# 0417keito/JEN-1-pytorch

Hardware: AMD Instinct MI355X
Metric: denoiser steps/sec (B=8, 128x1500 latents) (higher is better)
Workload: dtype bf16; 1 GPU; configs[1] full JEN-1 1D-UNet (296.5M params), B=8 per GPU, latents 128x1500, 100-step DDIM schedule, eta=1 (the reference's default, gdm.py:28: every step adds sigma * noise; the per-step noise is a table drawn before the timed region and READ inside it), no CFG (CFG dropout off: sampling), hipGraph-replayed step; per sampling run and outside the timed region: the text K/V projection and the time; global_batch=8, seq_len=1500, parallelism=replicas x1 (independent samples)

## Files before the change

### include/jen1_deep.h

```cpp
#ifndef JEN1_DEEP_H
#define JEN1_DEEP_H

#include <stdint.h>

#include "jen1_hip.h"

#ifdef __cplusplus
extern "C" {
#endif

#define JEN1_DEEP_GEMM 0
#define JEN1_DEEP_ATTN 1
#define JEN1_DEEP_STATS 2
#define JEN1_DEEP_TILE 3

#define JEN1_DEEP_MAX_SRC 4
#define JEN1_DEEP_MAX_SEG 12
#ifndef JEN1_DEEP_THREADS
#define JEN1_DEEP_THREADS 512
#endif
#define JEN1_DEEP_BLOB_BYTES 4096
#define JEN1_DEEP_MAX_PHASES 256
#ifndef JEN1_DEEP_SHARDS
#define JEN1_DEEP_SHARDS 32
// ... 38 lines not shown
  int32_t pro_mode, norm_C, gn_groups, gn_cpg, gran;
  float inv_count, gn_eps, inv_vpr, inv_Lin, inv_Lout, inv_groups;
  int32_t p_ld;
  int32_t lvn, lvr;
  int32_t out_C, ps_f, ps_off, L_y, y_brows, y_row0, ld_y, ld_res, act, y_f32;
  int32_t part_off, stat_off, red_off;
  jen1_deep_src src[JEN1_DEEP_MAX_SRC];
  int32_t red_bytes;
  int32_t Lp, Hb, zrow, Rtot;
  int32_t lS, lvpg, lgroups;
  int32_t mrep;
  int32_t live_mask;
  const float* wscale;
  int32_t n_chunks, Lc;
  float inv_nchunks;
  int32_t pad_hot_;
  const float* edge_bias;
} jen1_deep_hot;

typedef struct jen1_deep_tile {
  const float* st[2];
  float* out_part;
  int32_t st_tiles[2], st_nfg[2];
  int32_t st_live;
  int32_t cmain;
  int32_t taps, pad_left;
  int32_t tb, tiles_t;
  int32_t BM, mblocks, MF;
  int32_t NF, KS, kch, rows_in;
  int32_t out_nfg, out_cps;
  int32_t tab_off, red_off;
// ... 25 lines not shown
} jen1_deep_phase;

int jen1_deep_phase_size(void);
int jen1_deep_has_chunks(void);

int jen1_deep_phase_conv(const jen1_conv_args* a, int nb_max, jen1_deep_phase* out);

int jen1_deep_phase_attention(const void* q, const void* k, const void* v, void* out_t, const int32_t* kv_row, const void* kv_extra,
                              const int32_t* extra_row, const int32_t* extra_step, int ld_extra, int kx_off, int vx_off, int B, int H,
                              int d, int Nq, int Nk, int ldq, int q_off, int ldkv, int k_off, int v_off, int ldo, int causal,
                              float scale, const float* ln_u, const float* ln_b, int ln_C, float ln_eps, int finish_q,
                              int finish_kv, int kv_live , int dtype, jen1_deep_phase* out);

int jen1_deep_phase_stats(const void* x, float* stats, int B, int L, int ld, int dtype, jen1_deep_phase* out);

int jen1_deep_phase_tile(const jen1_conv_args* a, int tb, int bm, const float* st0, int st0_tiles, int st0_nfg, const float* st1,
                         int st1_tiles, int st1_nfg, int st_live, float* out_part, int out_nfg, jen1_deep_phase* out);
int jen1_deep_tile_count(int L_out, int tb, int M, int bm);

int jen1_deep_link(jen1_deep_phase* phases, int n_phases, int nwg, void* blobs, void* headers);
int jen1_deep_blob_bytes(void);

int jen1_deep_poison(const void* table_dev, int n, uint32_t* sync, void* stream);
int jen1_deep_poison_zero(const void* table_dev, int n, uint32_t* sync, void* zero_ptr, int64_t zero_bytes, void* stream);

int64_t jen1_deep_sync_bytes(int n_phases);

int jen1_deep_num_workgroups(void);

int jen1_deep_run(const void* blobs_dev, const void* headers_dev, int n_phases, uint32_t* sync, int nwg, int lds_bytes, int dtype,
// ... 14 lines not shown
```

### include/jen1_hip.h

```cpp
#ifndef JEN1_HIP_H
#define JEN1_HIP_H

#include <stdint.h>

#ifdef __cplusplus
extern "C" {
#endif

#define JEN1_F32 0
#define JEN1_BF16 1
#define JEN1_FP8 2

#define JEN1_PRO_NONE 0
#define JEN1_PRO_GN 1
#define JEN1_PRO_GN_SILU 2
#define JEN1_PRO_LN 3
#define JEN1_PRO_SILU 4

#define JEN1_ACT_NONE 0
#define JEN1_ACT_GELU 1

#define JEN1_CFG_W64x64 0
#define JEN1_CFG_W128x64 1
#define JEN1_CFG_S16x64 2
// ... 58 lines not shown
  int32_t splitk;
  int32_t cfg;
  int32_t direct;
  const void* zeros;
  int32_t tiles_t;
  float inv_tiles_t, inv_tb;
  const int32_t* film_step;
  const float* ln_u;
  int32_t ln_fold;
  int32_t nseg;
  jen1_conv_seg seg[JEN1_MAX_SEG];
  int32_t m_split;
  int32_t k_split;
  const float* w_scale;
  int32_t live_mask;
  int32_t reserved_;
  const float* edge_bias;
} jen1_conv_args;

int jen1_conv_gemm(const jen1_conv_args* args, void* stream);
int64_t jen1_conv_gemm_lds_bytes(const jen1_conv_args* args);
int jen1_cfg_bm(int cfg);
int jen1_cfg_bn(int cfg);

typedef struct jen1_norm_args {
  const void* x0; const void* x1; void* y;
  const float* gn_stats0; const float* gn_stats1;
  const float* gamma; const float* beta;
  const float* film; const int32_t* film_row;
  const float* ln_rowstats;
  int32_t dtype, mode, B, L, c0, c1, ld0, ld1, ld_y;
// ... 168 lines not shown
```

### jen-1-pytorch_amd/csrc/deep_kernel.hip

```cpp
#include <cstdlib>
#include <type_traits>
#ifdef JEN1_DEEP_EXP_PLAIN
#define JEN1_LIVE_LOAD(p) (*(p))
#endif
#include "live_words.h"
#include "mfma_frag.h"
#include "jen1_deep.h"

namespace {

constexpr int NT = JEN1_DEEP_THREADS;
constexpr int NW = NT / 64;
constexpr int SHARDS = JEN1_DEEP_SHARDS;
static_assert(SHARDS >= 1 && SHARDS <= 63, "one wave polls the shards and the error word");
constexpr int SHW = JEN1_DEEP_SHARD_WORDS;
constexpr int QCHUNK = 32;
#ifndef JEN1_DEEP_ATTN_LIVE_VEC
#define JEN1_DEEP_ATTN_LIVE_VEC 2
#endif

template <typename T> struct Mode { typedef T G; };
template <> struct Mode<fp8_t> { typedef bf16_t G; };
constexpr float P_SCALE = JEN1_FP8_P_SCALE;

// ... 1933 lines not shown
  JEN1_CHECK(!a->ln_fold && !a->row_scale, "deep conv: LayerNorm-fold epilogue / row scale are not supported by the persistent kernel");
  JEN1_CHECK(a->c0 > 0 && a->c0 % 32 == 0 && a->c1 % 32 == 0 && a->M % 16 == 0, "deep conv: channels must be multiples of 32, M of 16");
  JEN1_CHECK(a->taps >= 1 && a->stride >= 1 && a->B >= 1 && a->L_in >= 1 && a->L_out >= 1, "deep conv: bad geometry");
  JEN1_CHECK(a->nseg >= 0 && a->nseg <= JEN1_DEEP_MAX_SRC - 2, "deep conv: at most %d extra K segments", JEN1_DEEP_MAX_SRC - 2);
  JEN1_CHECK(a->taps + a->nseg <= JEN1_DEEP_MAX_SEG, "deep conv: too many K segments");
  const int es = a->dtype == JEN1_F32 ? 4 : (a->dtype == JEN1_FP8 ? 1 : 2);
  const int maxv = a->dtype == JEN1_F32 ? JEN1_DEEP_MAXV_F : JEN1_DEEP_MAXV_B;
  jen1_deep_phase& p = *out;
  memset(&p, 0, sizeof(p));
  p.h.wscale = a->dtype == JEN1_FP8 ? a->w_scale : nullptr;
  p.h.live_mask = a->live_mask;
  p.h.kind = JEN1_DEEP_GEMM;
  p.h.dtype = a->dtype;
  p.h.dep = -1;
  int ns = 0, coff = 0;
  p.h.src[ns++] = jen1_deep_src{a->x0, a->ld0, a->c0, 0, 1.0f};
  coff = a->c0;
  if (a->c1) {
    JEN1_CHECK(a->x1, "deep conv: c1 without x1");
    p.h.src[ns++] = jen1_deep_src{a->x1, a->ld1, a->c1, coff, a->src1_scale};
    coff += a->c1;
  }
  const int cmain = coff;
  int G = 0, nseg = 0;
  for (int tap = 0; tap < a->taps; ++tap) {
    G += cmain / 32;
    p.seg[nseg++] = jen1_deep_seg{0, tap - a->pad_left, G, 0};
  }
  for (int s = 0; s < a->nseg; ++s) {
    const jen1_conv_seg& e = a->seg[s];
    JEN1_CHECK(e.x && e.kch > 0 && e.ld >= 32 * e.kch, "deep conv: bad extra segment %d", s);
// ... 189 lines not shown
  jen1_deep_phase& p = *out;
  memset(&p, 0, sizeof(p));
  p.h.kind = JEN1_DEEP_STATS;
  p.h.dtype = dtype;
  p.h.dep = -1;
  p.sx = x; p.sstats = stats; p.sL = L; p.sld = ld;
  p.scpf = ld / JEN1_FINE_GROUPS;
  p.sgran = p.scpf >= 8 ? 8 : p.scpf;
  p.h.B = B;
  p.h.n_units = B;
  const int vpr = ld / 8, sub = 8 / p.sgran;
  p.h.lds_bytes = align16i((JEN1_DEEP_THREADS / vpr) * vpr * sub * 8);
  return 0;
}

extern "C" int jen1_deep_tile_count(int L_out, int tb, int M, int bm) {
  if (tb < 1 || bm < 1) return 0;
  return ceil_div(L_out, tb) * ceil_div(M, bm);
}

extern "C" int jen1_deep_phase_tile(const jen1_conv_args* a, int tb, int bm, const float* st0, int st0_tiles, int st0_nfg, const float* st1,
                                    int st1_tiles, int st1_nfg, int st_live, float* out_part, int out_nfg, jen1_deep_phase* out) {
  JEN1_CHECK(a && out, "deep tile: null pointer");
  JEN1_CHECK(a->dtype == JEN1_F32 || a->dtype == JEN1_BF16, "deep tile: dtype must be float32 or bf16 (the JEN1_FP8 mode runs the long levels in bf16)");
  JEN1_CHECK(a->x0 && a->w && a->y, "deep tile: null tensor");
  JEN1_CHECK(!a->edge_bias, "deep tile: an edge bias is an option of the deep GEMM phases only");
  JEN1_CHECK(a->pro_mode == JEN1_PRO_NONE || a->pro_mode == JEN1_PRO_GN || a->pro_mode == JEN1_PRO_GN_SILU, "deep tile: prologue %d is not supported", a->pro_mode);
  JEN1_CHECK(!a->ln_fold && !a->row_scale && !a->out_rowstats && a->act == JEN1_ACT_NONE && a->m_split == 0, "deep tile: LayerNorm / row scale / activation / dual range are not tile options");
  JEN1_CHECK(a->c0 > 0 && a->c0 % 32 == 0 && a->c1 % 32 == 0 && a->M % 16 == 0, "deep tile: channels must be multiples of 32, M of 16");
  JEN1_CHECK(a->taps >= 1 && a->stride >= 1 && a->B >= 1 && a->L_in >= 1 && a->L_out >= 1, "deep tile: bad geometry");
// ... 96 lines not shown
  p.tl.tab_off = tile_b;
  p.tl.red_off = tile_b + align16i(8 * cmain);
  const int tot = p.tl.red_off + (2 * (JEN1_DEEP_THREADS / 64) * 64 + 128) * 4;
  JEN1_CHECK(tot <= LDS_BUDGET, "deep tile: %d B of LDS", tot);
  p.h.lds_bytes = tot;
  p.h.n_units = p.tl.mblocks * a->B * p.tl.tiles_t;
  JEN1_CHECK(p.h.n_units < (1 << 20), "deep tile: too many units");
  p.tl.inv_tiles_t = 1.0f / (float)p.tl.tiles_t;
  p.tl.inv_bt = 1.0f / (float)(a->B * p.tl.tiles_t);
  p.h.inv_vpr = 1.0f / (float)(coff / 8);
  p.h.inv_Lin = 1.0f / (float)a->L_in;
  p.h.inv_Lout = 1.0f / (float)a->L_out;
  return 0;
}

extern "C" int jen1_deep_link(jen1_deep_phase* phases, int n_phases, int nwg, void* blobs, void* headers) {
  JEN1_CHECK(phases && blobs && headers && n_phases >= 1 && nwg >= 1, "deep link: bad arguments");
  JEN1_CHECK(n_phases <= JEN1_DEEP_MAX_PHASES, "deep link: %d phases (at most %d)", n_phases, JEN1_DEEP_MAX_PHASES);
  int lds = 0, rot = 0, units_before = 0;
  unsigned char* bl = reinterpret_cast<unsigned char*>(blobs);
  int32_t* hd = reinterpret_cast<int32_t*>(headers);
  memset(bl, 0, (size_t)n_phases * BLOB);
  for (int p = 0; p < n_phases; ++p) {
    jen1_deep_phase& P = phases[p];
    if (P.h.kind == JEN1_DEEP_GEMM && P.h.mrep == 1 && !getenv("JEN1_DEEP_NO_MREP")) {
      int mrep = 1;
      const char* cap_s = getenv("JEN1_DEEP_UNIT_CAP");
      int cap = cap_s ? atoi(cap_s) : nwg;
      static const int cap_attn = getenv("JEN1_DEEP_CAP_BEFORE_ATTN") ? atoi(getenv("JEN1_DEEP_CAP_BEFORE_ATTN")) : 0;
      if (cap_attn > 0 && p + 1 < n_phases && phases[p + 1].h.kind == JEN1_DEEP_ATTN && cap_attn < cap) cap = cap_attn;
      const int nch = P.h.n_chunks < 1 ? 1 : P.h.n_chunks;
      while (mrep < 8 && (P.h.MT / mrep) * P.h.groups_n * nch > cap && P.h.MT % (2 * mrep) == 0 && P.h.mt_split % (2 * mrep) == 0) mrep *= 2;
      if (mrep > 1 && P.h.lds_bytes + P.h.red_bytes <= LDS_BUDGET) {
        P.h.mrep = mrep;
        P.h.n_units = (P.h.MT / mrep) * P.h.groups_n * nch;
        P.h.lds_bytes += P.h.red_bytes;
      }
    }
    P.h.dep = p - 1;
    P.h.dep_units = p ? phases[p - 1].h.n_units : 0;
    P.h.rot = rot % nwg;
    rot += ((P.h.n_units + 7) / 8) * 8;
    lds = P.h.lds_bytes > lds ? P.h.lds_bytes : lds;
    unsigned char* b = bl + (size_t)p * BLOB;
    memcpy(b, &P, sizeof(P));
    hd[4 * p + 0] = P.h.n_units; hd[4 * p + 1] = P.h.rot; hd[4 * p + 2] = P.h.kind; hd[4 * p + 3] = units_before;
    units_before += P.h.n_units;
    if (P.h.kind != JEN1_DEEP_GEMM) continue;
    int16_t* cnt = reinterpret_cast<int16_t*>(b + TAB_OFF);
    int32_t* runs = reinterpret_cast<int32_t*>(b + TAB_OFF + 64);
    const int tmax = (P.h.L_out - 1) * P.h.stride;
    int k0 = 0;
    for (int s = 0; s < P.h.nseg; ++s) {
      const int sb = s ? P.seg[s - 1].gend : 0, se = P.seg[s].gend, sh = P.seg[s].shift;
      if (!(tmax + sh >= 0 && sh < P.h.L_in)) continue;
      const bool low = P.h.mt_split && sb < P.h.g_split;
      JEN1_CHECK(!low || se <= P.h.g_split, "deep link: phase %d: the dual-range split must fall on a segment boundary", p);
      const int Ls = se - sb;
      for (int w = 0; w < NW; ++w) {
        const int i0 = ((w - k0) % NW + NW) % NW;
        if (i0 >= Ls) continue;
        const int n = (Ls - i0 + NW - 1) / NW;
        const int r = cnt[2 * NW + w];
        JEN1_CHECK(r < MAXRUN, "deep link: phase %d has more than %d runs per wave", p, MAXRUN);
        int32_t* e = runs + ((size_t)w * MAXRUN + r) * 4;
        e[0] = sb + i0; e[1] = n; e[2] = P.seg[s].coff + i0 * 32; e[3] = sh;
        cnt[w] = (int16_t)(cnt[w] + n);
        cnt[2 * NW + w] = (int16_t)(r + 1);
        if (low) { cnt[NW + w] = cnt[w]; cnt[3 * NW + w] = cnt[2 * NW + w]; }
      }
      k0 += Ls;
    }
    if (!P.h.mt_split) for (int w = 0; w < NW; ++w) { cnt[NW + w] = cnt[w]; cnt[3 * NW + w] = cnt[2 * NW + w]; }
    const int pf = P.h.dtype == JEN1_F32 ? JEN1_DEEP_PF_F : JEN1_DEEP_PF_B;
    int32_t* slots = reinterpret_cast<int32_t*>(b + SLOT_OFF);
    int32_t* curs = reinterpret_cast<int32_t*>(b + CUR_OFF);
    for (int w = 0; w < NW; ++w) {
      const int32_t* rw = runs + (size_t)w * MAXRUN * 4;
      const int nr = cnt[2 * NW + w], tot = cnt[w];
// ... 8 lines not shown
        if (i + 1 == pf) {
          int r2 = r, l2 = left, g2 = g, c2 = col, s2 = sh;
          if (i + 1 < tot) {
            if (--l2 > 0) { g2 += NW; c2 += NW * 32; }
            else if (r2 + 1 < nr) { ++r2; l2 = rw[r2 * 4 + 1]; g2 = rw[r2 * 4]; c2 = rw[r2 * 4 + 2]; s2 = rw[r2 * 4 + 3]; }
          }
          curs[w * 8 + 0] = r2; curs[w * 8 + 1] = l2; curs[w * 8 + 2] = g2; curs[w * 8 + 3] = c2; curs[w * 8 + 4] = s2;
        }
        if (i + 1 < tot) next();
      }
    }
  }
  return lds + WS_OFF;
}

namespace {
struct PoisonEntry {
  unsigned long long ptr, bytes;
};
__global__ __launch_bounds__(256) void poison_kernel(const PoisonEntry* __restrict__ tab, unsigned* __restrict__ sync, int n_tab, void* zero_ptr,
                                                      unsigned long long zero_bytes) {
  if ((int)blockIdx.y >= n_tab) {
    uint4* z = reinterpret_cast<uint4*>(zero_ptr);
    const size_t n = zero_bytes >> 4;
    const size_t nblk = (size_t)gridDim.x * (gridDim.y - n_tab), blk = (size_t)(blockIdx.y - n_tab) * gridDim.x + blockIdx.x;
    for (size_t i = blk * 256 + threadIdx.x; i < n; i += nblk * 256) z[i] = make_uint4(0u, 0u, 0u, 0u);
    return;
  }
  const PoisonEntry e = tab[blockIdx.y];
  uint4* p = reinterpret_cast<uint4*>(e.ptr);
// ... 90 lines not shown
```

### jen-1-pytorch_amd/jen1_amd/engine.py

```python
from __future__ import annotations

import contextlib
import ctypes as C
import math
import weakref
import os
import time
from collections import namedtuple
from typing import Callable, Dict, List, Optional, Tuple

import torch

from . import lib as L
from .config import ResSpec, TransformerSpec, UNetSpec
from .packing import (conv_weight_to_gemm, convT_weight_to_gemm, ff_out_matrix, fold_layernorm, fold_linear_into_upsample,
                      o1q2_matrix, o2f1_matrix, pack_gemm_weight, pqkv_matrix, s1q2_matrix)

FG = 32


def _ceil_to(x: int, m: int) -> int:
    return (x + m - 1) // m * m


# ... 163 lines not shown

    def nbytes(self) -> int:
        return sum(t.numel() * t.element_size() for t in self.w.values())

    def fold_up(self, uname: str) -> Tuple[torch.Tensor, torch.Tensor, torch.Tensor]:
        key = f"{uname}.upf"
        if key not in self.w:
            f, wt, b_up, wp, bp, w2, b2 = self._fold_src[uname]
            wm, bm = ff_out_matrix(wp, bp, w2, b2)
            wf, b_mid, b_first, b_last = fold_linear_into_upsample(wt, b_up, f, wm, bm)
            self.w[key] = pack_gemm_weight(wf, self.dtype)
            self.v[f"{key}.bias"] = b_mid.float().contiguous()
            self.v[f"{key}.edge"] = torch.stack([b_first, b_last], 0).float().contiguous()
        return self.w[key], self.v[f"{key}.bias"], self.v[f"{key}.edge"]

    def fp8(self, w: torch.Tensor) -> Tuple[torch.Tensor, torch.Tensor]:
        hit = self._fp8.get(id(w))
        if hit is not None and hit[0] is w:
            return hit[1], hit[2]
        MT = w.shape[-3]
        wf = w.reshape(-1, MT, 4, 16, 8).to(torch.float32)
        amax = wf.abs().amax(dim=(0, 2, 4))
        scale = (amax / 448.0).clamp_min(1e-20)
        q = (wf / scale[None, :, None, :, None]).to(torch.float8_e4m3fn).view(torch.uint8).reshape(-1, MT, 64, 8).contiguous()
        scale = scale.reshape(-1).contiguous()
        self._fp8[id(w)] = (w, q, scale)
        return q, scale


def _bgemm_parts(groups):
    if all(n0 % 128 == 0 and N % 128 == 0 for _, _, n0, N, _ in groups):
        return [groups]
    return [[gr] for gr in groups]


def _group_align(part) -> int:
    n_lo = part[0][2]
    return 256 if all((n0 - n_lo) % 256 == 0 and N % 256 == 0 for _, _, n0, N, _ in part) else 128


def parse_fold_up(s: str) -> Optional[frozenset]:
    s = s.strip().lower()
    if s in ("", "1", "all", "on"):
        return None
    if s in ("0", "off", "none"):
        return frozenset()
    return frozenset(int(v) for v in s.split(",") if v.strip())


class DeepIneligible(Exception):
    """a layer does not fit the persistent deep-level kernel (LDS / staging registers / unsupported option)"""


class DeepProgram:

    _static_owner: Dict[str, "weakref.ref"] = {}

    def __init__(self, eng, leader: Optional["DeepProgram"] = None, err: Optional[torch.Tensor] = None):
# ... 62 lines not shown
    def _new(self):
        return (C.c_char * self.dsize)()

    def _add(self, buf, rc, label, out, kind="gemm", part=None):
        if rc != 0:
            msg = self.lib.jen1_last_error()
            raise self.ineligible(f"{label}: {msg.decode() if msg else 'does not fit'}")
        self.bufs.append(buf)
        self.labels.append(label)
        self.outs.append(out)
        self.kinds.append(kind)
        self._note_output(out)
        if part is not None:
            self._produced.setdefault(part.untyped_storage().data_ptr(), part)

    def add_conv(self, a: "L.ConvArgs", label: str, out, nb_max: int = 0):
        buf = self._new()
        self._add(buf, self.lib.jen1_deep_phase_conv(C.byref(a), nb_max, C.cast(buf, C.c_void_p)), label, out)

    def add_tile(self, a: "L.ConvArgs", tb: int, bm: int, st, out_part, out_nfg: int, label: str, out):
        buf = self._new()
        st = list(st) + [None] * (2 - len(st))
        p = [(0, 0, 0) if e is None else (e[0], e[1], e[2]) for e in st]
        live = sum(1 << k for k, e in enumerate(st) if e is not None and e[3])
        rc = self.lib.jen1_deep_phase_tile(C.byref(a), tb, bm, p[0][0] or None, p[0][1], p[0][2], p[1][0] or None, p[1][1], p[1][2], live,
                                           _ptr(out_part), out_nfg, C.cast(buf, C.c_void_p))
        self._add(buf, rc, label, out, kind="tile", part=out_part)

    def add_attention(self, args, label: str, out):
        buf = self._new()
        self._add(buf, self.lib.jen1_deep_phase_attention(*args, C.cast(buf, C.c_void_p)), label, out, kind="attn")

    def add_stats(self, x: "Act", stats: torch.Tensor, label: str):
# ... 138 lines not shown
    def __call__(self, stream: int) -> None:
        self.fn(stream)


def conv_traffic(taps: int, c_real: int, c_extra: int, M: int, B: int, L_in: int, L_out: int, L_y: int, out_C: int, *,
                 w_es: int, act_es: int, out_es: int, scale_bytes: int = 0) -> Tuple[int, int, int]:
    k = taps * c_real + c_extra
    return k * M * w_es + scale_bytes, B * L_in * (c_real + c_extra) * act_es + B * L_y * out_C * out_es, 2 * k * M * B * L_out


def _extras_fit_tile(extra_segs, padded_ok: bool = False) -> bool:
    return len(extra_segs) <= 2 and all(sh == 0 and (padded_ok or e.cp == e.C) and e.cp % 32 == 0 for e, sh in extra_segs)


class ConvRequest(namedtuple("ConvRequest", "ops src0 src1 w bias edge_bias out pro gn film ln act residual row_scale y_f32 extra_segs m_split k_split "
                                            "flat_w taps out_C force label")):
    __slots__ = ()
    normed = property(lambda self: [s for s in (self.src0, self.src1) if s is not None] if self.pro in (L.PRO_GN, L.PRO_GN_SILU) else [])
    sources = property(lambda self: [s for s in (self.src0, self.src1) if s is not None] + [e for e, _ in self.extra_segs])
    k_extra = property(lambda self: sum(e.cp for e, _ in self.extra_segs))


class KernelCtx:

    def __init__(self, dtype: str = "f32", device="cuda", target_wgs: int = 256):
        self.lib = L.load()
        self.device = torch.device(device)
        self.dt = L.F32 if dtype == "f32" else L.BF16
        self.tdtype = torch.float32 if dtype == "f32" else torch.bfloat16
        self.deep_dt = self.dt
        self.target_wgs = target_wgs
# ... 50 lines not shown
                      trace=bool(os.environ.get("JEN1_DEBUG_SYNC")))

    def _run_ops(self, ops, stream: Optional[int], trace: bool = False):
        if stream is None:
            stream = torch.cuda.current_stream(self.eng.device).cuda_stream
        for i, op in enumerate(ops if trace else ()):
            print(f"[jen1] op {i}: {getattr(op, 'label', '') or '?'}", flush=True)
            op(stream)
            torch.cuda.synchronize(self.eng.device)
        for op in (() if trace else ops):
            op(stream)

    def conv(self, ops, *, src0: Act, w: torch.Tensor, bias, out: Act, taps=1, stride=1, pad_left=0, L_out=None,
             src1: Optional[Act] = None, src1_scale=1.0, ps_f=1, ps_off=0, L_y=None, y_row0=0, pro=L.PRO_NONE,
             gn=None, film=None, ln=None, act=L.ACT_NONE, residual: Optional[Act] = None, row_scale=None,
             y_f32=False, out_C=None, force=None, label="", extra_segs=None, m_split=0, k_split=0, flat_w=False, edge_bias=None):
        rq = ConvRequest(ops, src0, src1, w, bias, edge_bias, out, pro, gn, film, ln, act, residual, row_scale, y_f32, extra_segs or [],
                         m_split, k_split, flat_w, taps, out_C if out_C is not None else out.C, force, label)
        a = self._conv_args(rq, stride, pad_left, L_out, src1_scale, ps_f, ps_off, L_y, y_row0)
        if self._long_on:
            return self._conv_long(a, rq)
        if self._deep_on:
            return self._conv_deep(a, rq)
        if src0.L in self.tile_lens and not self.det:
            try:
                return self._conv_tile(L.ConvArgs.from_buffer_copy(a), rq)
            except DeepIneligible as e:
                self.tile_errors.append(str(e))
        return self._conv_launch(a, rq)

    def _conv_args(self, rq: ConvRequest, stride, pad_left, L_out, src1_scale, ps_f, ps_off, L_y, y_row0) -> "L.ConvArgs":
        src0, src1, w, out, pro, taps, label = rq.src0, rq.src1, rq.w, rq.out, rq.pro, rq.taps, rq.label
        a = L.ConvArgs()
        a.x0, a.c0, a.ld0 = src0.t.data_ptr(), src0.cp, src0.ld
# ... 81 lines not shown
        eng, out, label = self.eng, rq.out, rq.label
        if rq.pro == L.PRO_LN or rq.y_f32 or rq.row_scale is not None:
            raise DeepIneligible(f"{label}: prologue / epilogue option outside the persistent kernel")
        if out.ld != out.C:
            raise DeepIneligible(f"{label}: {out.C} output channels are not a multiple of 32 (padding columns would stay poisoned)")
        a.out_gn_stats = a.out_rowstats = None
        w8 = None
        if eng.deep_dt == L.FP8:
            w8 = eng.W.fp8(rq.w)
            a.dtype, a.w, a.w_scale = L.FP8, w8[0].data_ptr(), w8[1].data_ptr()
        self._film2(a, rq)
        self._fill_segs(a, rq.extra_segs, shifts=True, padded_ok=False)
        a.live_mask = self._live_mask(self.deep, rq)
        if rq.m_split:
            a.m_split, a.k_split = rq.m_split, rq.k_split
        self._keep.append((a, rq, w8))
        self.deep.add_conv(a, f"conv[{label}] B={a.B} Lin={a.L_in} Lout={a.L_out} c0={a.c0} c1={a.c1} taps={a.taps} M={a.M}", out,
                           nb_max=self._deep_nb_cap(a, rq, 1 if w8 is not None else (4 if eng.dt == L.F32 else 2)))
        self._traffic(a, rq, self.deep, w_es=1 if w8 is not None else None, scale_bytes=4 * a.M if w8 is not None else 0)
        out.gn_valid = False
        return out

    def _deep_nb_cap(self, a: "L.ConvArgs", rq: ConvRequest, w_es: int) -> int:
        eng = self.eng
        nb_cap = eng.deep_nb_max
        if eng.deep_unit_target > 0:
            wbytes = (rq.taps * (a.c0 + a.c1) + rq.k_extra) * a.M * w_es
            nb = 1
            while nb < a.B and ((a.M // 16) * -(-a.B // nb) > eng.deep_unit_target or -(-a.B // nb) * wbytes > eng.deep_reread_cap):
                nb *= 2
            nb_cap = nb if nb_cap == 0 else min(nb_cap, nb)
        return nb_cap

# ... 356 lines not shown
        self.use_long = bool(deep and eng.use_deep and eng.use_long and not self.tile_lens)
        self.long_errors: List[str] = []
        while True:
            super().__init__(eng)
            self.progs: List[DeepProgram] = []
            self._deep_prog: Optional[DeepProgram] = None
            self._deep_err = None
            self.time_ops: List[Callable[[int], None]] = []
            self.ctx_ops: List[Callable[[int], None]] = []
            self.pack_ops: List[Callable[[int], None]] = []
            self.pack_rows = None
            self.poison_op, self.poison_args = None, None
            self.taps: Dict[str, Act] = {}
            self.fold_errors: List[str] = []
            self.folded_levels: List[int] = []
            self.acts: List[Act] = []
            self.n_launch = 0
            self.deep_level = first if first < n_lv else None
            try:
                self._build()
                break
            except LongIneligible as e:
                self.long_errors.append(str(e))
                self.use_long = False
            except DeepIneligible as e:
                self.deep_errors.append(f"level {first}: {e}")
                if first >= n_lv:
                    assert self.tile_lens, f"persistent launch: {e}"
                    self.tile_lens = frozenset()
                else:
# ... 59 lines not shown
        self._deep_on = False

    def _prog_close(self, need_totals=()):
        prog = self._prog
        assert prog is not None and len(prog) > 0
        for x in need_totals:
            prog.add_stats(x, x.gn, f"stats B={x.B} L={x.L} ld={x.ld}")
            x.gn_valid = True
        self._prog = None
        self._deep_on = False
        self._emit_program(prog, "deep")

    def take_error(self) -> int:
        return self.progs[0].take_error() if self.progs else 0

    def resblock(self, r: ResSpec, src0: Act, src1: Optional[Act], causal: bool, gn=True) -> Act:
        W, ops = self.eng.W, self.ops
        n = r.name
        sc = self.eng.skip_scale if src1 is not None else 1.0
        pad = 2 if causal else 1
        h = self.new_act(src0.B, src0.L, r.c_out, gn=True)
        self.conv(ops, src0=src0, src1=src1, src1_scale=sc, w=W.w[f"{n}.conv1"], bias=W.v[f"{n}.conv1.bias"], out=h,
                  taps=3, pad_left=pad, pro=L.PRO_GN_SILU,
                  gn=(r.groups, r.c_in, W.v[f"{n}.gn1.g"], W.v[f"{n}.gn1.b"], 1e-5))
        y = self.new_act(src0.B, src0.L, r.c_out, gn=gn)
        gn2 = (r.groups, r.c_out, W.v[f"{n}.gn2.g"], W.v[f"{n}.gn2.b"], 1e-5)
        film = (self.film, self.film_row, W.film_off[n], r.c_out, self.step_idx if (self.table_mode and not self.per_sample) else None)
        srcs_raw = [src0] + ([src1] if src1 is not None else [])
        if r.has_shortcut and self.eng.fuse_shortcut and f"{n}.conv2s" in W.w \
                and (self._long_on or all(s_.cp == s_.C for s_ in srcs_raw)) and 3 + len(srcs_raw) <= L.MAX_SEG:
            try:
                if self.conv(ops, src0=h, w=W.w[f"{n}.conv2s"], bias=W.v[f"{n}.conv2s.bias"], out=y, taps=3, pad_left=pad,
                             pro=L.PRO_GN_SILU, gn=gn2, film=film, extra_segs=[(s_, 0) for s_ in srcs_raw]) is not None:
                    return y
            except DeepIneligible:
                if not (self._deep_on or self._long_on):
                    raise
        if r.has_shortcut:
            res = self.new_act(src0.B, src0.L, r.c_out)
            self.conv(ops, src0=src0, src1=src1, src1_scale=1.0, w=W.w[f"{n}.short"], bias=W.v[f"{n}.short.bias"], out=res)
        else:
            assert src1 is None
            res = src0
        self.conv(ops, src0=h, w=W.w[f"{n}.conv2"], bias=W.v[f"{n}.conv2.bias"], out=y, taps=3, pad_left=pad,
                  pro=L.PRO_GN_SILU, gn=gn2, film=film, residual=res)
        return y

    def transformer(self, t: TransformerSpec, x: Act, causal: bool, fold_out: bool = False, list_out: bool = True):
        W, ops, eng = self.eng.W, self.ops, self.eng
        n, Cc, H, d = t.name, t.channels, t.heads, t.head_features
        mid = H * d
        Bf, Lx = x.B, x.L
        gn_in = (32, Cc, W.v[f"{n}.gn.g"], W.v[f"{n}.gn.b"], 1e-6)
        kv = self.kv_ctx[n]
        xattn = dict(kv_t=kv, ldkv=2 * mid, k_off=0, v_off=mid, H=H, d=d, Nk=eng.spec.ctx_len, causal=False, kv_row=self.kv_row,
                     kv_extra=self.kvx.t if eng.spec.use_xattn_time else None,
                     extra_row=self.extra_row if eng.spec.use_xattn_time else None, ld_extra=W.kvx_ld,
                     kx_off=W.kvx_off[n], vx_off=W.kvx_off[n] + mid,
                     extra_step=self.step_idx if (self.table_mode and eng.spec.use_xattn_time) else None)
        fold1 = (eng.fold_single_position and Lx == 1 and eng.fuse_ln_proj and self.streams(Bf, Lx, Cc) and Cc % 256 == 0 and mid % 32 == 0
# ... 237 lines not shown
                skips.append(x)
            if d.transformer:
                x = self.transformer(d.transformer, x, causal)
                skips.append(x)
            skips_list.append(skips)
            self.taps[f"down{i}"] = x
        x = self.resblock(spec.bott_pre, x, None, causal)
        if spec.bott_tr:
            x = self.transformer(spec.bott_tr, x, causal)
        x = self.resblock(spec.bott_post, x, None, causal)
        self.taps["bottleneck"] = x
        for idx, u in enumerate(spec.ups):
            if use_long and n_lv - 1 - idx == self.long_levels - 1:
                self._long_begin()
            skips = skips_list.pop()
            for r in u.blocks:
                sk = skips.pop()
                assert x.L == sk.L, (x.L, sk.L)
                x = self.resblock(r, x, sk, causal)
            f = u.factor
            level = n_lv - 1 - idx
            xf = None
            if u.transformer:
                fold = self._deep_on and f > 1 and (eng.fold_up is None or level in eng.fold_up)
                x = self.transformer(u.transformer, x, causal, fold_out=fold, list_out=f == 1)
                if isinstance(x, tuple):
                    xf, x = x, x[0]
            last = idx == len(spec.ups) - 1
            L_need = skip0.L if last else (skips_list[-1][-1].L if skips_list[-1] else f * x.L)
            y = self.new_act(Be, L_need, u.c_out, gn=True)
            res = skip0 if last else None
            p, diff = f // 2 + f % 2, f * x.L - L_need
            assert diff >= 0
            if xf is not None:
                wf_, bf_, ef_ = W.fold_up(u.name)
                try:
# ... 183 lines not shown
        self.tile_min_rows = int(os.environ.get("JEN1_TILE_MIN_ROWS", "512"))
        self.tile_target_wgs = int(os.environ.get("JEN1_TILE_TARGET_WGS", "256"))
        self.tile_one_round = os.environ.get("JEN1_TILE_ONE_ROUND", "0") != "0"
        self.use_deep = os.environ.get("JEN1_DEEP", "1") != "0"
        self.use_long = os.environ.get("JEN1_LONG", "1") != "0"
        self.deep_all_slots = os.environ.get("JEN1_DEEP_ALL_SLOTS", "0") != "0"
        self.deterministic = os.environ.get("JEN1_DETERMINISTIC", "0") != "0"
        self.pack_fixed_order = os.environ.get("JEN1_PACK_FIXED_ORDER", "1") != "0"
        self.deep_max_len = int(os.environ.get("JEN1_DEEP_MAX_LEN", "64"))
        self.use_tile_phases = os.environ.get("JEN1_TILE_PHASES", "0") != "0"
        self.tile_phase_min_len = int(os.environ.get("JEN1_TILE_PHASE_MIN_LEN", "200"))
        self.deep_nb_max = int(os.environ.get("JEN1_DEEP_NB_MAX", "0"))
        self.deep_unit_target = int(os.environ.get("JEN1_DEEP_UNIT_TARGET", "128"))
        self.deep_reread_cap = int(float(os.environ.get("JEN1_DEEP_REREAD_MB", "16")) * (1 << 20))
        self.fold_up = parse_fold_up(os.environ.get("JEN1_FOLD_UP", "1"))
        self.plans: Dict[tuple, Plan] = {}
        self.load_params(params)

    def load_params(self, params: Dict[str, torch.Tensor]):
        self.W = Weights(self.spec, params, self.tdtype, self.device)
        self.plans.clear()
        self.kv_fixed: Dict[str, torch.Tensor] = {}
        self._project_fixed_embedding()

    def _stream(self) -> int:
        return torch.cuda.current_stream(self.device).cuda_stream

    def _project_fixed_embedding(self):
        spec, W = self.spec, self.W
        if not spec.transformers():
# ... 16 lines not shown
            n_lo, n_hi = part[0][2], part[-1][2] + part[-1][3]
            g.a, g.groups = fx.data_ptr(), tab.data_ptr()
            g.b = W.w["kv2_all"].data_ptr() + n_lo * F * W.w["kv2_all"].element_size()
            g.M, g.Ntot, g.K, g.lda, g.ldb, g.n_groups, g.dtype, g.alpha = n, n_hi - n_lo, F, F, F, len(part), self.dt, 1.0
            g.group_align = _group_align(part)
            L.check(lib.jen1_big_gemm(C.byref(g), s), "jen1_big_gemm")
        torch.cuda.synchronize(dev)

    def plan(self, B: int, T: int, nrep: int, causal: bool, slot: int = 0, n_t: Optional[int] = None,
             deep: Optional[bool] = None, deterministic: Optional[bool] = None, per_sample: bool = False) -> Plan:
        if deep is None:
            deep = slot == 0 or self.deep_all_slots
        deep = bool(deep) and self.use_deep
        det = self.deterministic if deterministic is None else bool(deterministic)
        per_sample = bool(per_sample) and n_t is not None and self.spec.context_features is not None
        key = (B, T, nrep, bool(causal), slot, n_t, deep, det, self.fold_up) + ((True,) if per_sample else ())
        if key not in self.plans:
            self.plans[key] = Plan(self, B, T, nrep, bool(causal), n_t, deep=deep, deterministic=det, per_sample=per_sample)
        return self.plans[key]
```

### jen-1-pytorch_amd/jen1_amd/lib.py

```python
from __future__ import annotations

import ctypes as C
import os
import subprocess
from typing import Optional

HERE = os.path.dirname(os.path.abspath(__file__))
PKG_ROOT = os.path.dirname(HERE)
REPO_ROOT = os.path.dirname(PKG_ROOT)
ABI_VERSION = 2
LIB_PATH = os.environ.get("JEN1_LIB", os.path.join(HERE, "libjen1_hip.so"))
CSRC = os.path.join(PKG_ROOT, "csrc")
INCLUDE = os.path.join(REPO_ROOT, "include")
SOURCES = ["conv_gemm.hip", "stream_gemm.hip", "tile_gemm.hip", "norm_apply.hip", "attention.hip", "deep_kernel.hip", "elementwise.hip",
           "optimizer.hip", "train_gemm.hip", "train_ops.hip", "train_attn.hip", "encodec.hip", "big_gemm.hip", "train_glue.hip", "train_kvbank.hip",
           "long_kernel.hip", "audio.hip", "t5.hip", "global_cond.hip", "windows.hip", "loudness.hip", "spectral.hip"]

F32, BF16, FP8 = 0, 1, 2
PRO_NONE, PRO_GN, PRO_GN_SILU, PRO_LN, PRO_SILU = 0, 1, 2, 3, 4
ACT_NONE, ACT_GELU = 0, 1
CFG_W64x64, CFG_W128x64, CFG_S16x64, CFG_S16x32, CFG_S16x16 = 0, 1, 2, 3, 4
CFG_T128x64, CFG_T128x32, CFG_T128x16, CFG_T256x32, CFG_T256x16, CFG_T64x64 = 5, 6, 7, 8, 9, 10
T5_ACT_GELU_NEW, T5_ACT_RELU, T5_MAX_TOKENS = 0, 1, 128
FORM_SCALAR, FORM_VECTOR, FORM_FUSED256, FORM_FUSED1024 = 0, 1, 2, 3
# ... 24 lines not shown
        ("dtype", c_int), ("B", c_int), ("L_in", c_int), ("L_out", c_int),
        ("c0", c_int), ("c1", c_int), ("ld0", c_int), ("ld1", c_int),
        ("taps", c_int), ("stride", c_int), ("pad_left", c_int),
        ("M", c_int), ("out_C", c_int), ("ps_f", c_int), ("ps_off", c_int),
        ("L_y", c_int), ("y_brows", c_int), ("y_row0", c_int), ("ld_y", c_int), ("ld_res", c_int),
        ("y_f32", c_int), ("pro_mode", c_int),
        ("gn_groups", c_int), ("gn_cpg", c_int), ("gn_count", c_int),
        ("gn_eps", c_float), ("src1_scale", c_float),
        ("film_off", c_int), ("film_C", c_int), ("film_ld", c_int),
        ("ln_C", c_int), ("ln_eps", c_float),
        ("act", c_int), ("out_cpf", c_int), ("tb", c_int), ("nb", c_int),
        ("kc_stage", c_int), ("splitk", c_int), ("cfg", c_int), ("direct", c_int),
        ("zeros", c_void_p), ("tiles_t", c_int), ("inv_tiles_t", c_float), ("inv_tb", c_float),
        ("film_step", c_void_p), ("ln_u", c_void_p), ("ln_fold", c_int), ("nseg", c_int),
        ("seg", ConvSeg * MAX_SEG), ("m_split", c_int), ("k_split", c_int), ("w_scale", c_void_p),
        ("live_mask", c_int), ("reserved_", c_int), ("edge_bias", c_void_p),
    ]


class NormArgs(C.Structure):
    _fields_ = [
        ("x0", c_void_p), ("x1", c_void_p), ("y", c_void_p), ("gn_stats0", c_void_p), ("gn_stats1", c_void_p),
        ("gamma", c_void_p), ("beta", c_void_p), ("film", c_void_p), ("film_row", c_void_p), ("ln_rowstats", c_void_p),
        ("dtype", c_int), ("mode", c_int), ("B", c_int), ("L", c_int), ("c0", c_int), ("c1", c_int),
        ("ld0", c_int), ("ld1", c_int), ("ld_y", c_int), ("groups", c_int), ("cpg", c_int), ("count", c_int),
        ("eps", c_float), ("src1_scale", c_float), ("film_off", c_int), ("film_C", c_int), ("film_ld", c_int),
        ("film_step", c_void_p),
    ]


class GemmOperand(C.Structure):
# ... 141 lines not shown
    "jen1_lstm_layer": (c_int, [_P, _P, _P, _P] + [c_int] * 5 + [_P]),
    "jen1_lstm_layer_multi": (c_int, [_P, _P, _P, _P, _P, _P] + [c_int] * 5 + [_P]),
    "jen1_codec_segment_scales": (c_int, [_P, _P, c_int, c_int, c_int64, c_int, c_int, c_int, _P]),
    "jen1_codec_segment_cut": (c_int, [_P, _P, _P, c_int, c_int, c_int64] + [c_int] * 6 + [_P]),
    "jen1_codec_pad1d": (c_int, [_P, _P] + [c_int] * 6 + [_P]),
    "jen1_codec_overlap_add": (c_int, [_P, c_int, _P, _P] + [c_int] * 8 + [_P]),
    "jen1_deep_phase_size": (c_int, []),
    "jen1_deep_has_chunks": (c_int, []),
    "jen1_deep_phase_conv": (c_int, [C.POINTER(ConvArgs), c_int, _P]),
    "jen1_deep_phase_attention": (c_int, [_P, _P, _P, _P, _P, _P, _P, _P, c_int, c_int, c_int] + [c_int] * 12 +
                                  [c_float, _P, _P, c_int, c_float, c_int, c_int, c_int, c_int, _P]),
    "jen1_deep_phase_stats": (c_int, [_P, _P, c_int, c_int, c_int, c_int, _P]),
    "jen1_deep_phase_tile": (c_int, [C.POINTER(ConvArgs), c_int, c_int, _P, c_int, c_int, _P, c_int, c_int, c_int, _P, c_int, _P]),
    "jen1_deep_tile_count": (c_int, [c_int, c_int, c_int, c_int]),
    "jen1_deep_link": (c_int, [_P, c_int, c_int, _P, _P]),
    "jen1_deep_poison": (c_int, [_P, c_int, _P, _P]),
    "jen1_deep_poison_zero": (c_int, [_P, c_int, _P, _P, c_int64, _P]),
    "jen1_deep_blob_bytes": (c_int, []),
    "jen1_deep_sync_bytes": (c_int64, [c_int]),
    "jen1_deep_num_workgroups": (c_int, []),
    "jen1_deep_run": (c_int, [_P, _P, c_int, _P, c_int, c_int, c_int, _P]),
    "jen1_deep_run_err": (c_int, [_P, _P, c_int, _P, _P, c_int, c_int, c_int, _P]),
    "jen1_deep_error_word": (c_int, [c_int]),
    "jen1_deep_run_mode": (c_int, [_P, _P, c_int, _P, _P, c_int, c_int, c_int, c_int, _P]),
    "jen1_deep_run_kinds": (c_int, [_P, _P, c_int, _P, _P, c_int, c_int, c_int, c_int, c_int, _P]),
    "jen1_long_geometry": (c_int, [c_int, c_int, c_int, C.POINTER(c_int), C.POINTER(c_int), C.POINTER(c_int)]),
    "jen1_long_phase_conv": (c_int, [C.POINTER(ConvArgs), c_int, _P, c_int, c_int, c_int, _P, c_int, c_int, c_int, c_int, _P, _P]),
    "jen1_long_phase_lds": (c_int, [_P]),
    "jen1_long_phase_units": (c_int, [_P]),
    "jen1_long_run": (c_int, [_P, c_int, c_int, _P, _P, c_int, c_int, c_int, c_int, _P]),
# ... 127 lines not shown
```

Baseline: 859.6 denoiser steps/s.

## Split skip-concat resblock conv1 into off-chain skip half and on-chain x half

```diff
diff --git a/include/jen1_deep.h b/include/jen1_deep.h
--- a/include/jen1_deep.h
+++ b/include/jen1_deep.h
@@ -76,7 +76,7 @@
   const float* wscale;
   int32_t n_chunks, Lc;
   float inv_nchunks;
-  int32_t pad_hot_;
+  int32_t off_chain;
   const float* edge_bias;
 } jen1_deep_hot;
 
@@ -132,6 +132,8 @@
 
 int jen1_deep_phase_stats(const void* x, float* stats, int B, int L, int ld, int dtype, jen1_deep_phase* out);
 
+int jen1_deep_phase_off_chain(jen1_deep_phase* ph, int on);
+
 int jen1_deep_phase_tile(const jen1_conv_args* a, int tb, int bm, const float* st0, int st0_tiles, int st0_nfg, const float* st1,
                          int st1_tiles, int st1_nfg, int st_live, float* out_part, int out_nfg, jen1_deep_phase* out);
 int jen1_deep_tile_count(int L_out, int tb, int M, int bm);
diff --git a/include/jen1_hip.h b/include/jen1_hip.h
--- a/include/jen1_hip.h
+++ b/include/jen1_hip.h
@@ -96,7 +96,7 @@
   int32_t k_split;
   const float* w_scale;
   int32_t live_mask;
-  int32_t reserved_;
+  float src0_scale;
   const float* edge_bias;
 } jen1_conv_args;
 
diff --git a/jen-1-pytorch_amd/csrc/deep_kernel.hip b/jen-1-pytorch_amd/csrc/deep_kernel.hip
--- a/jen-1-pytorch_amd/csrc/deep_kernel.hip
+++ b/jen-1-pytorch_amd/csrc/deep_kernel.hip
@@ -1971,7 +1971,7 @@
   p.h.dtype = a->dtype;
   p.h.dep = -1;
   int ns = 0, coff = 0;
-  p.h.src[ns++] = jen1_deep_src{a->x0, a->ld0, a->c0, 0, 1.0f};
+  p.h.src[ns++] = jen1_deep_src{a->x0, a->ld0, a->c0, 0, a->src0_scale != 0.0f ? a->src0_scale : 1.0f};
   coff = a->c0;
   if (a->c1) {
     JEN1_CHECK(a->x1, "deep conv: c1 without x1");
@@ -2191,6 +2191,13 @@
   return 0;
 }
 
+extern "C" int jen1_deep_phase_off_chain(jen1_deep_phase* ph, int on) {
+  JEN1_CHECK(ph, "deep off-chain: null pointer");
+  JEN1_CHECK(ph->h.kind == JEN1_DEEP_GEMM, "deep off-chain: only GEMM phases are placed off the chain");
+  ph->h.off_chain = on ? 1 : 0;
+  return 0;
+}
+
 extern "C" int jen1_deep_tile_count(int L_out, int tb, int M, int bm) {
   if (tb < 1 || bm < 1) return 0;
   return ceil_div(L_out, tb) * ceil_div(M, bm);
@@ -2317,9 +2324,54 @@
   return 0;
 }
 
+#define LINK_CHECK(cond, ...)                      \
+  do {                                             \
+    if (!(cond)) return -jen1_set_error(__VA_ARGS__); \
+  } while (0)
 extern "C" int jen1_deep_link(jen1_deep_phase* phases, int n_phases, int nwg, void* blobs, void* headers) {
-  JEN1_CHECK(phases && blobs && headers && n_phases >= 1 && nwg >= 1, "deep link: bad arguments");
-  JEN1_CHECK(n_phases <= JEN1_DEEP_MAX_PHASES, "deep link: %d phases (at most %d)", n_phases, JEN1_DEEP_MAX_PHASES);
+  LINK_CHECK(phases && blobs && headers && n_phases >= 1 && nwg >= 1, "deep link: bad arguments");
+  LINK_CHECK(n_phases <= JEN1_DEEP_MAX_PHASES, "deep link: %d phases (at most %d)", n_phases, JEN1_DEEP_MAX_PHASES);
+  {
+    struct Range { uintptr_t view_lo, lo, hi; };
+    Range out[JEN1_DEEP_MAX_PHASES];
+    auto esz = [](const jen1_deep_phase& P) { return (uintptr_t)(P.h.dtype == JEN1_F32 ? 4 : 2); };
+    for (int p = 0; p < n_phases; ++p) {
+      const jen1_deep_phase& P = phases[p];
+      out[p] = Range{0, 0, 0};
+      if (P.h.kind == JEN1_DEEP_GEMM || P.h.kind == JEN1_DEEP_TILE) {
+        const uintptr_t y = reinterpret_cast<uintptr_t>(P.h.y), ey = P.h.y_f32 ? 4 : esz(P), pitch_b = (uintptr_t)P.h.ld_y * ey;
+        out[p] = Range{y >= pitch_b ? y - pitch_b + ey : 0, y, y + (uintptr_t)P.h.B * (uintptr_t)P.h.y_brows * pitch_b};
+      } else if (P.h.kind == JEN1_DEEP_ATTN) {
+        const uintptr_t o = reinterpret_cast<uintptr_t>(P.out), pitch_b = (uintptr_t)P.ldo * esz(P);
+        out[p] = Range{o >= pitch_b ? o - pitch_b + esz(P) : 0, o, o + (uintptr_t)P.h.B * (uintptr_t)P.Nq * pitch_b};
+      }
+    }
+    auto late_producer = [&](int p, const void* ptr) {
+      const uintptr_t a = reinterpret_cast<uintptr_t>(ptr);
+      for (int q = 0; q < p; ++q)
+        if (a >= out[q].view_lo && a < out[q].hi) return -1;
+      for (int q = p + 1; q < n_phases; ++q)
+        if (a >= out[q].lo && a < out[q].hi) return q;
+      return -1;
+    };
+    for (int p = 0; p < n_phases; ++p) {
+      const jen1_deep_phase& P = phases[p];
+      if (P.h.kind == JEN1_DEEP_GEMM || P.h.kind == JEN1_DEEP_TILE) {
+        for (int k = 0; k < P.h.nsrc && k < JEN1_DEEP_MAX_SRC; ++k)
+          LINK_CHECK(!((P.h.live_mask >> k) & 1) || late_producer(p, P.h.src[k].x) < 0,
+                     "deep link: phase %d polls source %d, which phase %d writes: a producer must come first in program order", p, k,
+                     late_producer(p, P.h.src[k].x));
+        LINK_CHECK(!((P.h.live_mask >> 8) & 1) || !P.h.residual || late_producer(p, P.h.residual) < 0,
+                   "deep link: phase %d polls its residual, which phase %d writes: a producer must come first in program order", p,
+                   late_producer(p, P.h.residual));
+      } else if (P.h.kind == JEN1_DEEP_ATTN) {
+        LINK_CHECK(!(P.kv_live & 1) || (late_producer(p, P.k) < 0 && late_producer(p, P.v) < 0),
+                   "deep link: phase %d polls its keys / values, which a later phase writes: a producer must come first in program order", p);
+        LINK_CHECK(!(P.kv_live & 2) || late_producer(p, P.q) < 0,
+                   "deep link: phase %d polls its queries, which a later phase writes: a producer must come first in program order", p);
+      }
+    }
+  }
   int lds = 0, rot = 0, units_before = 0;
   unsigned char* bl = reinterpret_cast<unsigned char*>(blobs);
   int32_t* hd = reinterpret_cast<int32_t*>(headers);
@@ -2343,7 +2395,7 @@
     P.h.dep = p - 1;
     P.h.dep_units = p ? phases[p - 1].h.n_units : 0;
     P.h.rot = rot % nwg;
-    rot += ((P.h.n_units + 7) / 8) * 8;
+    if (!P.h.off_chain) rot += ((P.h.n_units + 7) / 8) * 8;
     lds = P.h.lds_bytes > lds ? P.h.lds_bytes : lds;
     unsigned char* b = bl + (size_t)p * BLOB;
     memcpy(b, &P, sizeof(P));
@@ -2358,14 +2410,14 @@
       const int sb = s ? P.seg[s - 1].gend : 0, se = P.seg[s].gend, sh = P.seg[s].shift;
       if (!(tmax + sh >= 0 && sh < P.h.L_in)) continue;
       const bool low = P.h.mt_split && sb < P.h.g_split;
-      JEN1_CHECK(!low || se <= P.h.g_split, "deep link: phase %d: the dual-range split must fall on a segment boundary", p);
+      LINK_CHECK(!low || se <= P.h.g_split, "deep link: phase %d: the dual-range split must fall on a segment boundary", p);
       const int Ls = se - sb;
       for (int w = 0; w < NW; ++w) {
         const int i0 = ((w - k0) % NW + NW) % NW;
         if (i0 >= Ls) continue;
         const int n = (Ls - i0 + NW - 1) / NW;
         const int r = cnt[2 * NW + w];
-        JEN1_CHECK(r < MAXRUN, "deep link: phase %d has more than %d runs per wave", p, MAXRUN);
+        LINK_CHECK(r < MAXRUN, "deep link: phase %d has more than %d runs per wave", p, MAXRUN);
         int32_t* e = runs + ((size_t)w * MAXRUN + r) * 4;
         e[0] = sb + i0; e[1] = n; e[2] = P.seg[s].coff + i0 * 32; e[3] = sh;
         cnt[w] = (int16_t)(cnt[w] + n);
@@ -2404,6 +2456,8 @@
   return lds + WS_OFF;
 }
 
+#undef LINK_CHECK
+
 namespace {
 struct PoisonEntry {
   unsigned long long ptr, bytes;
diff --git a/jen-1-pytorch_amd/jen1_amd/engine.py b/jen-1-pytorch_amd/jen1_amd/engine.py
--- a/jen-1-pytorch_amd/jen1_amd/engine.py
+++ b/jen-1-pytorch_amd/jen1_amd/engine.py
@@ -201,6 +201,17 @@
             self.v[f"{key}.edge"] = torch.stack([b_first, b_last], 0).float().contiguous()
         return self.w[key], self.v[f"{key}.bias"], self.v[f"{key}.edge"]
 
+    def split_skip(self, n: str, C: int) -> Tuple[torch.Tensor, ...]:
+        key = f"{n}.conv1.x"
+        if key not in self.w:
+            w, g, b = self.w[f"{n}.conv1"], self.v[f"{n}.gn1.g"], self.v[f"{n}.gn1.b"]
+            assert w.shape[1] * 32 == 2 * C and g.numel() == 2 * C, (n, tuple(w.shape), C)
+            self.w[key], self.w[f"{n}.conv1.s"] = w[:, : C // 32].contiguous(), w[:, C // 32:].contiguous()
+            for h, sl in (("x", slice(0, C)), ("s", slice(C, 2 * C))):
+                self.v[f"{n}.gn1.g.{h}"], self.v[f"{n}.gn1.b.{h}"] = g[sl].contiguous(), b[sl].contiguous()
+        return (self.w[key], self.w[f"{n}.conv1.s"], self.v[f"{n}.gn1.g.x"], self.v[f"{n}.gn1.b.x"], self.v[f"{n}.gn1.g.s"],
+                self.v[f"{n}.gn1.b.s"])
+
     def fp8(self, w: torch.Tensor) -> Tuple[torch.Tensor, torch.Tensor]:
         hit = self._fp8.get(id(w))
         if hit is not None and hit[0] is w:
@@ -229,6 +240,21 @@
 def parse_fold_up(s: str) -> Optional[frozenset]:
     s = s.strip().lower()
     if s in ("", "1", "all", "on"):
+        return None
+    if s in ("0", "off", "none"):
+        return frozenset()
+    return frozenset(int(v) for v in s.split(",") if v.strip())
+
+
+SPLIT_SKIP_DEFAULT = frozenset({7})
+SPLIT_SKIP_AUTO = "auto"
+
+
+def parse_split_skip(s: str):
+    s = s.strip().lower()
+    if s in ("", "1", "on", "auto"):
+        return SPLIT_SKIP_AUTO
+    if s == "all":
         return None
     if s in ("0", "off", "none"):
         return frozenset()
@@ -321,9 +347,18 @@
         if part is not None:
             self._produced.setdefault(part.untyped_storage().data_ptr(), part)
 
-    def add_conv(self, a: "L.ConvArgs", label: str, out, nb_max: int = 0):
+    def add_conv(self, a: "L.ConvArgs", label: str, out, nb_max: int = 0, off_chain: bool = False):
         buf = self._new()
-        self._add(buf, self.lib.jen1_deep_phase_conv(C.byref(a), nb_max, C.cast(buf, C.c_void_p)), label, out)
+        rc = self.lib.jen1_deep_phase_conv(C.byref(a), nb_max, C.cast(buf, C.c_void_p))
+        if rc == 0 and off_chain:
+            rc = self.lib.jen1_deep_phase_off_chain(C.cast(buf, C.c_void_p), 1)
+        self._add(buf, rc, label, out)
+
+    def probe_conv_units(self, a: "L.ConvArgs", nb_max: int = 0) -> int:
+        buf = self._new()
+        if self.lib.jen1_deep_phase_conv(C.byref(a), nb_max, C.cast(buf, C.c_void_p)) != 0:
+            return 0
+        return int(C.c_int32.from_buffer(buf, 4).value)
 
     def add_tile(self, a: "L.ConvArgs", tb: int, bm: int, st, out_part, out_nfg: int, label: str, out):
         buf = self._new()
@@ -492,7 +527,7 @@
 
 
 class ConvRequest(namedtuple("ConvRequest", "ops src0 src1 w bias edge_bias out pro gn film ln act residual row_scale y_f32 extra_segs m_split k_split "
-                                            "flat_w taps out_C force label")):
+                                            "flat_w taps out_C force label off_chain probe")):
     __slots__ = ()
     normed = property(lambda self: [s for s in (self.src0, self.src1) if s is not None] if self.pro in (L.PRO_GN, L.PRO_GN_SILU) else [])
     sources = property(lambda self: [s for s in (self.src0, self.src1) if s is not None] + [e for e, _ in self.extra_segs])
@@ -573,10 +608,15 @@
     def conv(self, ops, *, src0: Act, w: torch.Tensor, bias, out: Act, taps=1, stride=1, pad_left=0, L_out=None,
              src1: Optional[Act] = None, src1_scale=1.0, ps_f=1, ps_off=0, L_y=None, y_row0=0, pro=L.PRO_NONE,
              gn=None, film=None, ln=None, act=L.ACT_NONE, residual: Optional[Act] = None, row_scale=None,
-             y_f32=False, out_C=None, force=None, label="", extra_segs=None, m_split=0, k_split=0, flat_w=False, edge_bias=None):
+             y_f32=False, out_C=None, force=None, label="", extra_segs=None, m_split=0, k_split=0, flat_w=False, edge_bias=None,
+             src0_scale=1.0, off_chain=False, probe=False):
         rq = ConvRequest(ops, src0, src1, w, bias, edge_bias, out, pro, gn, film, ln, act, residual, row_scale, y_f32, extra_segs or [],
-                         m_split, k_split, flat_w, taps, out_C if out_C is not None else out.C, force, label)
+                         m_split, k_split, flat_w, taps, out_C if out_C is not None else out.C, force, label, off_chain, probe)
         a = self._conv_args(rq, stride, pad_left, L_out, src1_scale, ps_f, ps_off, L_y, y_row0)
+        assert (src0_scale == 1.0 and not off_chain and not probe) or self._deep_on, \
+            f"{label}: a scaled first source / an off-chain phase / a probe exist only in the persistent deep-level kernel"
+        if src0_scale != 1.0:
+            a.src0_scale = float(src0_scale)
         if self._long_on:
             return self._conv_long(a, rq)
         if self._deep_on:
@@ -688,9 +728,12 @@
         a.live_mask = self._live_mask(self.deep, rq)
         if rq.m_split:
             a.m_split, a.k_split = rq.m_split, rq.k_split
+        nb_max = self._deep_nb_cap(a, rq, 1 if w8 is not None else (4 if eng.dt == L.F32 else 2))
+        if rq.probe:
+            return self.deep.probe_conv_units(a, nb_max)
         self._keep.append((a, rq, w8))
         self.deep.add_conv(a, f"conv[{label}] B={a.B} Lin={a.L_in} Lout={a.L_out} c0={a.c0} c1={a.c1} taps={a.taps} M={a.M}", out,
-                           nb_max=self._deep_nb_cap(a, rq, 1 if w8 is not None else (4 if eng.dt == L.F32 else 2)))
+                           nb_max=nb_max, off_chain=rq.off_chain)
         self._traffic(a, rq, self.deep, w_es=1 if w8 is not None else None, scale_bytes=4 * a.M if w8 is not None else 0)
         out.gn_valid = False
         return out
@@ -1077,6 +1120,8 @@
             self.taps: Dict[str, Act] = {}
             self.fold_errors: List[str] = []
             self.folded_levels: List[int] = []
+            self.split_levels: List[int] = []
+            self.split_blocks = 0
             self.acts: List[Act] = []
             self.n_launch = 0
             self.deep_level = first if first < n_lv else None
@@ -1166,12 +1211,18 @@
     def take_error(self) -> int:
         return self.progs[0].take_error() if self.progs else 0
 
-    def resblock(self, r: ResSpec, src0: Act, src1: Optional[Act], causal: bool, gn=True) -> Act:
+    def resblock(self, r: ResSpec, src0: Act, src1: Optional[Act], causal: bool, gn=True, split=False) -> Act:
         W, ops = self.eng.W, self.ops
         n = r.name
         sc = self.eng.skip_scale if src1 is not None else 1.0
         pad = 2 if causal else 1
         h = self.new_act(src0.B, src0.L, r.c_out, gn=True)
+        if split and self._deep_on and src1 is not None and r.has_shortcut and r.groups % 2 == 0 and src0.C == src1.C == r.c_out \
+                and src0.cp == src0.C and src1.cp == src1.C and f"{n}.short" in W.w:
+            if split != SPLIT_SKIP_AUTO or 2 * self.conv(ops, src0=src0, src1=src1, src1_scale=sc, w=W.w[f"{n}.conv1"], bias=W.v[f"{n}.conv1.bias"],
+                                                        out=h, taps=3, pad_left=pad, pro=L.PRO_GN_SILU, probe=True,
+                                                        gn=(r.groups, r.c_in, W.v[f"{n}.gn1.g"], W.v[f"{n}.gn1.b"], 1e-5)) > self.deep.nwg:
+                return self._resblock_split(r, src0, src1, pad, gn, h)
         self.conv(ops, src0=src0, src1=src1, src1_scale=sc, w=W.w[f"{n}.conv1"], bias=W.v[f"{n}.conv1.bias"], out=h,
                   taps=3, pad_left=pad, pro=L.PRO_GN_SILU,
                   gn=(r.groups, r.c_in, W.v[f"{n}.gn1.g"], W.v[f"{n}.gn1.b"], 1e-5))
@@ -1196,6 +1247,25 @@
             res = src0
         self.conv(ops, src0=h, w=W.w[f"{n}.conv2"], bias=W.v[f"{n}.conv2.bias"], out=y, taps=3, pad_left=pad,
                   pro=L.PRO_GN_SILU, gn=gn2, film=film, residual=res)
+        return y
+
+    def _resblock_split(self, r: ResSpec, x: Act, skip: Act, pad: int, gn: bool, h: Act) -> Act:
+        W, ops, n, C_ = self.eng.W, self.ops, r.name, r.c_out
+        w1x, w1s, gx, bx, gs, bs = W.split_skip(n, C_)
+        g2 = r.groups // 2
+        s1 = self.new_act(x.B, x.L, C_, listed=False)
+        self.conv(ops, src0=skip, src0_scale=self.eng.skip_scale, w=w1s, bias=None, out=s1, taps=3, pad_left=pad, pro=L.PRO_GN_SILU,
+                  gn=(g2, C_, gs, bs, 1e-5), label="skip.s1 off-chain", off_chain=True)
+        self.conv(ops, src0=x, w=w1x, bias=W.v[f"{n}.conv1.bias"], out=h, taps=3, pad_left=pad, pro=L.PRO_GN_SILU,
+                  gn=(g2, C_, gx, bx, 1e-5), residual=s1, label="skip.conv1x")
+        sc = self.new_act(x.B, x.L, C_, listed=False)
+        self.conv(ops, src0=x, src1=skip, src1_scale=1.0, w=W.w[f"{n}.short"], bias=W.v[f"{n}.short.bias"], out=sc,
+                  label="skip.sc off-chain", off_chain=True)
+        y = self.new_act(x.B, x.L, C_, gn=gn)
+        film = (self.film, self.film_row, W.film_off[n], C_, self.step_idx if (self.table_mode and not self.per_sample) else None)
+        self.conv(ops, src0=h, w=W.w[f"{n}.conv2"], bias=W.v[f"{n}.conv2.bias"], out=y, taps=3, pad_left=pad, pro=L.PRO_GN_SILU,
+                  gn=(r.groups, C_, W.v[f"{n}.gn2.g"], W.v[f"{n}.gn2.b"], 1e-5), film=film, residual=sc, label="skip.conv2")
+        self.split_blocks += 1
         return y
 
     def transformer(self, t: TransformerSpec, x: Act, causal: bool, fold_out: bool = False, list_out: bool = True):
@@ -1463,12 +1533,20 @@
             if use_long and n_lv - 1 - idx == self.long_levels - 1:
                 self._long_begin()
             skips = skips_list.pop()
+            level = n_lv - 1 - idx
+            split = False
+            if self._deep_on and eng.split_skip == SPLIT_SKIP_AUTO:
+                split = SPLIT_SKIP_AUTO if (level in SPLIT_SKIP_DEFAULT and Be <= eng.split_skip_max_batch) else False
+            elif self._deep_on:
+                split = eng.split_skip is None or level in eng.split_skip
+            n_split = self.split_blocks
             for r in u.blocks:
                 sk = skips.pop()
                 assert x.L == sk.L, (x.L, sk.L)
-                x = self.resblock(r, x, sk, causal)
+                x = self.resblock(r, x, sk, causal, split=split)
+            if self.split_blocks > n_split:
+                self.split_levels.append(level)
             f = u.factor
-            level = n_lv - 1 - idx
             xf = None
             if u.transformer:
                 fold = self._deep_on and f > 1 and (eng.fold_up is None or level in eng.fold_up)
@@ -1682,6 +1760,8 @@
         self.deep_unit_target = int(os.environ.get("JEN1_DEEP_UNIT_TARGET", "128"))
         self.deep_reread_cap = int(float(os.environ.get("JEN1_DEEP_REREAD_MB", "16")) * (1 << 20))
         self.fold_up = parse_fold_up(os.environ.get("JEN1_FOLD_UP", "1"))
+        self.split_skip = parse_split_skip(os.environ.get("JEN1_SPLIT_SKIP", "1"))
+        self.split_skip_max_batch = int(os.environ.get("JEN1_SPLIT_SKIP_MAX_BATCH", "8"))
         self.plans: Dict[tuple, Plan] = {}
         self.load_params(params)
 
@@ -1728,7 +1808,7 @@
         deep = bool(deep) and self.use_deep
         det = self.deterministic if deterministic is None else bool(deterministic)
         per_sample = bool(per_sample) and n_t is not None and self.spec.context_features is not None
-        key = (B, T, nrep, bool(causal), slot, n_t, deep, det, self.fold_up) + ((True,) if per_sample else ())
+        key = (B, T, nrep, bool(causal), slot, n_t, deep, det, self.fold_up, self.split_skip, self.split_skip_max_batch) + ((True,) if per_sample else ())
         if key not in self.plans:
             self.plans[key] = Plan(self, B, T, nrep, bool(causal), n_t, deep=deep, deterministic=det, per_sample=per_sample)
         return self.plans[key]
diff --git a/jen-1-pytorch_amd/jen1_amd/lib.py b/jen-1-pytorch_amd/jen1_amd/lib.py
--- a/jen-1-pytorch_amd/jen1_amd/lib.py
+++ b/jen-1-pytorch_amd/jen1_amd/lib.py
@@ -62,7 +62,7 @@
         ("zeros", c_void_p), ("tiles_t", c_int), ("inv_tiles_t", c_float), ("inv_tb", c_float),
         ("film_step", c_void_p), ("ln_u", c_void_p), ("ln_fold", c_int), ("nseg", c_int),
         ("seg", ConvSeg * MAX_SEG), ("m_split", c_int), ("k_split", c_int), ("w_scale", c_void_p),
-        ("live_mask", c_int), ("reserved_", c_int), ("edge_bias", c_void_p),
+        ("live_mask", c_int), ("src0_scale", c_float), ("edge_bias", c_void_p),
     ]
 
 
@@ -234,6 +234,7 @@
     "jen1_deep_phase_tile": (c_int, [C.POINTER(ConvArgs), c_int, c_int, _P, c_int, c_int, _P, c_int, c_int, c_int, _P, c_int, _P]),
     "jen1_deep_tile_count": (c_int, [c_int, c_int, c_int, c_int]),
     "jen1_deep_link": (c_int, [_P, c_int, c_int, _P, _P]),
+    "jen1_deep_phase_off_chain": (c_int, [_P, c_int]),
     "jen1_deep_poison": (c_int, [_P, c_int, _P, _P]),
     "jen1_deep_poison_zero": (c_int, [_P, c_int, _P, _P, c_int64, _P]),
     "jen1_deep_blob_bytes": (c_int, []),
```

Result: no change. 866.6 denoiser steps/s, median of 6 (+0.8%).
